# BUTSpeechFIT/DiariZen

Hardware: AMD Instinct MI355X
Metric: audio-seconds/s (RTF) for wavlm-large-s80 pipeline, 16 kHz mono (higher is better)
Workload: dtype f32 (operands split into 2 fp16 terms with exact power-of-two scaling = 22 significant bits, 3 fp16 MFMA products, fp32 accumulate: the error-corrected '3xFP16/3xTF32' scheme; kernels without an fp16 variant use the 3-term bf16 split)

## Files before the change

### diarizen_amd/_lib.py

```python
from __future__ import annotations

import ctypes as C
import os
from pathlib import Path

DZN_MAX_CONV = 8
DZN_MAX_LAYERS = 32
DZN_MAX_HEADS = 16

DZN_PREC_F32 = 0
DZN_PREC_BF16 = 1
DZN_PREC_F32_SPLIT = 2
DZN_PREC_F32_H2 = 3
DZN_PREC_F16 = 4

DZN_ACT_NONE, DZN_ACT_GELU, DZN_ACT_SWISH, DZN_ACT_RELU = 0, 1, 2, 3

DZN_F32, DZN_F64, DZN_I64 = 0, 1, 2

ERRORS = {0: "ok", -1: "invalid argument", -2: "out of memory", -3: "HIP runtime error",
          -4: "bad call order", -5: "missing state_dict key"}


class DznError(RuntimeError):
# ... 174 lines not shown
    sig("dzn_op_amax", i32, [vp, i64, vp, vp])
    sig("dzn_op_split_rows", i32, [vp, vp, i64, i64, i32, vp])
    sig("dzn_op_conv3x3_c32", i32, [vp, vp, vp, vp, vp, i32, i32, i32, i32, i32, vp])
    sig("dzn_op_resblock_ws", i32, [vp, vp, vp, vp, vp, vp, vp, vp, vp, f32, f32, i32, i32, i32, i32, vp])
    sig("dzn_op_resblock32_fused", i32, [vp, vp, vp, vp, vp, vp, vp, vp, vp, f32, f32, i32, i32, i32, vp])
    sig("dzn_op_set_resblock_np", i32, [i32])
    sig("dzn_op_set_attention_noskip", i32, [i32])
    sig("dzn_op_conv3x3_c32_h2", i32, [vp, vp, vp, vp, vp, vp, vp, vp, i32, i32, i32, i32, i32, vp])
    sig("dzn_op_conv3x3_c32_ex", i32, [vp, vp, vp, vp, vp, vp, vp, vp, i32, i32, i32, i32, i32, vp, vp, vp, vp])
    sig("dzn_op_resblock32_fused_ex", i32, [vp, vp, vp, vp, vp, vp, vp, vp, vp, vp, f32, f32, i32, i32, i32, i32, vp, vp, vp])
    sig("dzn_op_resblock_ws_ex", i32, [vp, vp, vp, vp, vp, vp, vp, vp, vp, vp, f32, f32, i32, i32, i32, i32, i32, vp, vp, vp])
    sig("dzn_op_layernorm", i32, [vp, i64, vp, i64, vp, vp, i64, i32, i32, f32, i32, vp])
    sig("dzn_op_gate", i32, [vp, i64, vp, vp, vp, vp, i64, i32, vp])
    sig("dzn_op_row_stats", i32, [vp, i64, i64, i32, f32, vp, vp])
    sig("dzn_op_gate_stats", i32, [vp, i64, vp, vp, vp, vp, vp, vp, vp, i64, i32, f32, vp])
    sig("dzn_op_attention_h2", i32, [vp, vp, vp, vp, vp, i32, i32, i32, i32, i32, i32, f32, vp, vp])
    sig("dzn_op_set_attention_qb", i32, [i32])
    sig("dzn_op_set_attention_prefetch", i32, [i32])
    sig("dzn_op_attention_planes", i32, [vp, vp, vp, vp, vp, i32, i32, i32, i32, i32, i32, f32, vp, vp, vp, vp])
    sig("dzn_op_attention", i32, [vp, vp, vp, vp, vp, i32, i32, i32, i32, i32, i32, f32, i32, vp])
    sig("dzn_op_glu_dwconv", i32, [vp, i64, vp, vp, vp, i64, i32, i32, i32, i32, vp])
    sig("dzn_op_classify", i32, [vp, i64, vp, vp, vp, i64, i32, i32, i32, vp, vp, vp, vp])
    sig("dzn_op_groupnorm_gelu", i32, [vp, vp, i32, i32, i32, i32, i64, vp, vp, f32, vp, vp, vp])
    sig("dzn_op_gn_stats_floats", i64, [i32, i32, i32, i32])
    sig("dzn_op_pad_rows", i32, [vp, vp, i32, i32, i32, i32, i32, vp])
    sig("dzn_op_ws_accum", i32, [vp, vp, f32, i32, i64, vp])
    sig("dzn_op_ws_sum", i32, [C.POINTER(vp), C.POINTER(f32), i32, vp, i64, vp])
    sig("dzn_op_col_scale", i32, [vp, i64, i32, i64, vp, vp])
    sig("dzn_op_layernorm_t", i32, [vp, i64, vp, i64, vp, vp, vp, i64, i32, i32, f32, i32, vp, i64, vp])
    sig("dzn_op_wave_stats", i32, [vp, i32, i32, f32, vp, vp])
# ... 3 lines not shown
    sig("dzn_op_log_cmn_gather", i32, [vp, i32, vp, i32, i32, i32, f32, vp])
    sig("dzn_op_stem_conv", i32, [vp, i32, i32, i32, i32, vp, vp, vp, vp, vp, vp, vp])
    sig("dzn_op_stats_pool", i32, [vp, i32, i32, i32, i32, vp, i32, i32, vp, vp, vp])
    sig("dzn_op_window_active", i32, [vp, i32, i32, vp, vp])
    sig("dzn_op_compact_active", i32, [vp, i32, vp, vp, vp, vp])
    _LIB = lib
    return lib


EXPORTED = [
    "dzn_create", "dzn_load_tensor", "dzn_finalize_weights", "dzn_num_frames",
    "dzn_segment_forward", "dzn_segment_forward_soft", "dzn_embed_forward", "dzn_embed_forward_strided", "dzn_prepare_masks", "dzn_speaker_count", "dzn_cluster_activations", "dzn_detect", "dzn_detect_range", "dzn_diarize_range", "dzn_speaker_scores", "dzn_debug_fetch", "dzn_embed_skip_stats", "dzn_num_ignored",
    "dzn_workspace_bytes", "dzn_last_error", "dzn_destroy", "dzn_version", "dzn_linkage_centroid", "dzn_cdist_cosine", "dzn_host_workspace_release",
    "dzn_host_workspace_bytes",
    "dzn_flac_info", "dzn_flac_decode", "dzn_resample", "dzn_resample_tile", "dzn_decode", "dzn_ingest_many", "dzn_gather_windows", "dzn_vbx_create", "dzn_vbx_stats", "dzn_vbx_estep", "dzn_vbx_gamma", "dzn_vbx_destroy",
    "dzn_op_gemm", "dzn_op_split_weights", "dzn_op_split_weights_h2", "dzn_op_split_weights_mx", "dzn_op_set_gemm_mx_cfg", "dzn_checked_status", "dzn_op_set_gemm_cfg", "dzn_op_amax", "dzn_op_conv3x3_c32", "dzn_op_conv3x3_c32_h2", "dzn_op_resblock32_fused", "dzn_op_resblock_ws", "dzn_op_set_resblock_np", "dzn_op_conv3x3_c32_ex", "dzn_op_resblock32_fused_ex", "dzn_op_resblock_ws_ex", "dzn_op_set_attention_noskip", "dzn_op_split_rows", "dzn_op_layernorm", "dzn_op_row_stats", "dzn_op_gate", "dzn_op_gate_stats", "dzn_op_attention", "dzn_op_attention_h2", "dzn_op_attention_planes", "dzn_op_set_attention_qb", "dzn_op_set_attention_prefetch",
    "dzn_profile_enable", "dzn_profile_collect", "dzn_profile_reserve", "dzn_op_relpos_bucket",
    "dzn_op_glu_dwconv", "dzn_op_classify", "dzn_op_groupnorm_gelu", "dzn_op_gn_stats_floats", "dzn_op_pad_rows", "dzn_op_ws_accum",
    "dzn_op_ws_sum", "dzn_op_col_scale", "dzn_op_layernorm_t", "dzn_op_wave_stats", "dzn_op_frame_prep", "dzn_op_power",
    "dzn_op_log_cmn", "dzn_op_log_cmn_gather", "dzn_op_stem_conv", "dzn_op_stats_pool", "dzn_op_window_active",
    "dzn_op_compact_active",
]


def profile_enable(on: bool) -> None:
    check(load().dzn_profile_enable(int(on)), None, "dzn_profile_enable")


def profile_reserve(n_events: int) -> None:
    check(load().dzn_profile_reserve(int(n_events)), None, "dzn_profile_reserve")

# ... 24 lines not shown
```

### diarizen_amd/csrc/attention.hip

```cpp
#include "common.h"

namespace {

template <bool BIAS>
__global__ __launch_bounds__(256) void attn_kernel(const float* __restrict__ qkv,
                                                   float* __restrict__ out,
                                                   const float* __restrict__ gate,
                                                   const float* __restrict__ table,
                                                   const int32_t* __restrict__ head_idx, int B,
                                                   int L, int h, int Htot, int ldqkv, int ldo,
                                                   float scale) {
  extern __shared__ __attribute__((aligned(16))) float smem_f[];
  float* sK = smem_f;
  float* sV = smem_f + 64 * 64;
  float* sT = smem_f + 2 * 64 * 64;

  const int tid = threadIdx.x, lane = tid & 63, wave = tid >> 6;
  const int lr = lane & 15, lq = lane >> 4;
  const int qt = blockIdx.x, j = blockIdx.y, b = blockIdx.z;
  const int64_t rowbase = (int64_t)b * L;
  const float* Qp = qkv + j * 64;
  const float* Kp = qkv + (h + j) * 64;
  const float* Vp = qkv + (2 * h + j) * 64;

// ... 256 lines not shown
        }
      }
      ta = dpp_add<0xB1, 0xF>(ta);
      ta = dpp_add<0x4E, 0xF>(ta);
      tb = dpp_add<0xB1, 0xF>(tb);
      tb = dpp_add<0x4E, 0xF>(tb);
      if (H < Htot && sub == 0) {
        const float ga = 1.0f / (1.0f + expf(-(ta + ba)));
        const float gb = 1.0f / (1.0f + expf(-(tb + bb)));
        gate[row * Htot + H] = ga * (gb * cst[H] - 1.0f) + 2.0f;
      }
    }
  }
}

}

int launch_gate_stats(const float* x, int64_t ldx, const float* gamma, const float* beta, const float* Wg,
                      const float* bg, const float* cst, float* gate, float* stats, int64_t rows, int Htot, float eps,
                      hipStream_t s) {
  if (rows <= 0) return DZN_OK;
  if (Htot < 1 || Htot > 16) return DZN_E_INVALID;
  int pid = prof_enabled() ? prof_begin(s, "gate_ln_stats", 0.0, (double)rows * Htot * 64 * 4.0) : -1;
  int64_t grid = cdiv64(rows, 4);
  grid = grid > 256 * 8 ? 256 * 8 : grid;
  hipLaunchKernelGGL(gate_stats_kernel<16>, dim3((unsigned)grid), dim3(256), 0, s, x, ldx, gamma, beta, Wg,
                     bg, cst, gate, stats, rows, Htot, eps);
  prof_end(pid, s);
  return hipGetLastError() == hipSuccess ? DZN_OK : DZN_E_HIP;
}
// ... 61 lines not shown
```

### diarizen_amd/csrc/common.h

```cpp
#pragma once
#include <hip/hip_runtime.h>
#include <stdint.h>
#include <math.h>
#include <string.h>
#include "../../include/dzn.h"
#include "../../include/dzn_ops.h"

typedef float f32x4 __attribute__((ext_vector_type(4)));
typedef __bf16 bf16x8 __attribute__((ext_vector_type(8)));
typedef __bf16 bf16x4 __attribute__((ext_vector_type(4)));
typedef unsigned short u16;

#define DZN_WAVE 64

template <int CTRL, int ROW_MASK>
__device__ __forceinline__ float dpp_add(float v) {
  const int t = __builtin_amdgcn_update_dpp(ROW_MASK == 0xF ? __float_as_int(v) : 0, __float_as_int(v), CTRL,
                                            ROW_MASK, 0xF, false);
  return v + __int_as_float(t);
}
__device__ __forceinline__ float wave_sum(float v) {
  v = dpp_add<0xB1, 0xF>(v);
  v = dpp_add<0x4E, 0xF>(v);
  v = dpp_add<0x124, 0xF>(v);
  v = dpp_add<0x128, 0xF>(v);
  v = dpp_add<0x142, 0xA>(v);
  v = dpp_add<0x143, 0xC>(v);
  return __int_as_float(__builtin_amdgcn_readlane(__float_as_int(v), 63));
}
__device__ __forceinline__ float wave_max(float v) {
#pragma unroll
  for (int o = 32; o > 0; o >>= 1) v = fmaxf(v, __shfl_xor(v, o, 64));
  return v;
}

__device__ __forceinline__ void track_amax_lane(float* tracker, float m) {
  if (m > 0.f) {
    const unsigned cur = __hip_atomic_load(reinterpret_cast<unsigned int*>(tracker), __ATOMIC_RELAXED, __HIP_MEMORY_SCOPE_AGENT);
    if (__float_as_uint(m) > cur) atomicMax(reinterpret_cast<unsigned int*>(tracker), __float_as_uint(m));
  }
}
__device__ __forceinline__ void track_amax(float* tracker, float wave_partial) {
  const float m = wave_max(wave_partial);
  if ((threadIdx.x & 63) == 0) track_amax_lane(tracker, m);
}

__device__ __forceinline__ float erf_as(float x) {
  const float ax = fabsf(x);
// ... 13 lines not shown
__device__ __forceinline__ float swishf_(float x) { return x * sigmoidf_(x); }

__device__ __forceinline__ float apply_act(float v, int act) {
  switch (act) {
    case DZN_ACT_GELU: return gelu_erf(v);
    case DZN_ACT_SWISH: return swishf_(v);
    case DZN_ACT_RELU: return fmaxf(v, 0.0f);
    default: return v;
  }
}

static inline bool prec_is_h2(int p) { return p == DZN_PREC_F32_H2 || p == DZN_PREC_F16; }
static inline bool prec_is_split(int p) { return p == DZN_PREC_F32_SPLIT || prec_is_h2(p); }

int launch_gemm(const dzn_gemm_desc& d, hipStream_t s);
int launch_gemm_split(const dzn_gemm_desc& d, hipStream_t s);
int launch_gemm_split_pre(const dzn_gemm_desc& d, hipStream_t s);
int launch_pad_rows_split3(const float* x, void* planes, int64_t plane_stride, int B, int L, int Lp, int pad, int D,
                           hipStream_t st, int cg = 0, int cgp = 0);
int launch_pad_rows_split2(const float* x, void* planes, int64_t plane_stride, int B, int L, int Lp, int pad, int D,
                           const float* amax, float* snapshot, hipStream_t st, int cg = 0, int cgp = 0);
int launch_split_weights(const float* W, int64_t rows, int K, int64_t ldw, void* W3, hipStream_t s);
int launch_split_weights_h2(const float* W, int64_t rows, int K, int64_t ldw, void* W2, float* col_scale, hipStream_t s);
int host_stage_stream(int device, hipStream_t* stream);
int host_state_lease(int device, size_t bytes, hipStream_t* stream, char** base);
void host_state_release(int device);
int launch_gemm_mx(const dzn_gemm_desc& d, hipStream_t s);
int launch_split_weights_mx(const float* W, int64_t rows, int K, int64_t ldw, void* Wmx, float* col_scale, hipStream_t s);
int launch_amax(const float* x, int64_t n, float* amax, hipStream_t s);
int launch_fill_u32(void* p, unsigned value, int64_t n, hipStream_t st);
int launch_stats_finalize(const float* partial, int64_t rows, int P, int C, float eps, float* stats, hipStream_t s);
int launch_layernorm(const float* x, int64_t ldx, float* y, int64_t ldy, const float* g,
                     const float* b, int64_t rows, int C, int Cpad, float eps, int gelu,
                     hipStream_t s);
int launch_layernorm_t(const float* x, int64_t ldx, float* y, int64_t ldy, const float* g, const float* b,
                       const float* post, int64_t rows, int C, int Cpad, float eps, int gelu, hipStream_t s,
                       float* amax = nullptr, int64_t amax_unit = 0);
int launch_row_stats(const float* x, int64_t ldx, int64_t rows, int C, float eps, float* stats, hipStream_t s);
int launch_gate_stats(const float* x, int64_t ldx, const float* gamma, const float* beta, const float* Wg,
                      const float* bg, const float* cst, float* gate, float* stats, int64_t rows, int Htot, float eps,
                      hipStream_t s);
int launch_wave_stats(const float* w, int B, int N, float eps, float* stats, hipStream_t s);
int launch_gate(const float* y, int64_t ldy, const float* Wg, const float* bg, const float* cst,
                float* gate, int64_t rows, int Htot, hipStream_t s);
int launch_attention_t(const float* qkv, float* out, const float* gate, const float* table,
                       const int32_t* head_idx, int B, int L, int h, int Htot, int ldqkv, int ldo,
                       float scale, hipStream_t s);
int launch_attention_split(const float* qkv, float* out, const float* gate, const float* table,
                           const int32_t* head_idx, int B, int L, int h, int Htot, int ldqkv, int ldo,
                           float scale, hipStream_t s, const float* amax = nullptr);
int launch_attention(const float* qkv, float* out, const float* gate, const float* table,
                     const int32_t* head_idx, int B, int L, int h, int Htot, int ldqkv, int ldo,
                     float scale, int precision, hipStream_t s);
int launch_attention_planes(const float* qkv, const void* planes, int64_t plane_stride, const float* kvs, int kv_ld, float* out,
                            const float* gate, const float* table, const int32_t* head_idx, int B, int L, int h, int Htot,
                            int ldqkv, int ldo, float scale, hipStream_t s, const float* amax);
// ... 122 lines not shown
```

### diarizen_amd/csrc/engine.cpp

```cpp
#include <algorithm>
#include <cmath>
#include <cstdio>
#include <cstdlib>
#include <map>
#include <set>
#include <stdexcept>
#include <string>
#include <vector>

#include "common.h"

#define HIPCHK(x)                                                                        \
  do {                                                                                   \
    hipError_t e_ = (x);                                                                 \
    if (e_ != hipSuccess) {                                                              \
      throw EngineError(e_ == hipErrorOutOfMemory ? DZN_E_NOMEM : DZN_E_HIP,             \
                        std::string(#x) + ": " + hipGetErrorString(e_));                 \
    }                                                                                    \
  } while (0)

namespace {

struct EngineError : std::runtime_error {
  int code;
// ... 27 lines not shown
struct NormLin {
  LNp ln;
  Lin lin;
  bool folded = false;
};

struct EncLayer {
  bool attn = false, ffn = false;
  bool pre_norm = false;
  int h = 0, F = 0, Fp = 0;
  LNp ln1, ln2;
  NormLin qkv, f1;
  Lin out, f2;
  float *Wg = nullptr, *bg = nullptr, *cst = nullptr;
  int32_t* head_idx = nullptr;
};

struct ConfLayer {
  NormLin ffn1_w1, ffn2_w1, qkv, pw1;
  Lin ffn1_w2, ffn2_w2, o, pw2;
  LNp out_ln;
  float *dw = nullptr, *dwb = nullptr;
};

struct ResConv {
  Lin l;
  int cin = 0, cout = 0, ksz = 3, stride = 1;
  int k2 = 0;
  float l1max = 0.f, bmax = 0.f;
};
// ... 483 lines not shown
        h->rel_embed = e.v;
      }
    }
    if (L.ffn) {
      L.F = c.ffn_dim[i];
      L.Fp = pad32(L.F);
      maxF = std::max(maxF, L.Fp);
      L.f1 = norm_lin_from_sd(h, lp + ".feed_forward.intermediate_dense", L.pre_norm ? lp + ".final_layer_norm" : "", fold, L.F, D,
                              L.Fp, D, &L.ln2);
      L.f2 = linear_from_sd(h, lp + ".feed_forward.output_dense", D, L.F, D, L.Fp);
    }
  }
  if (h->rel_embed.empty())
    throw EngineError(DZN_E_INVALID, "layer 0 must carry attention (rel_attn_embed lives there)");
  {
    const HostT& w = need(h, "weight_sum.weight");
    expect_numel(w, c.n_layers + 1, "weight_sum.weight");
    h->wsum_w = w.v;
  }
  const int A = h->A, Fh = h->Fh;
  h->proj = linear_from_sd(h, "proj", A, D, A, D);
  h->lnorm = ln_from_sd(h, "lnorm", A);
  h->conf.resize(c.conf_layers);
  for (int i = 0; i < c.conf_layers; ++i) {
    ConfLayer& L = h->conf[i];
    const std::string cp = "conformer.conformer_layer." + std::to_string(i);
    L.ffn1_w1 = norm_lin_from_sd(h, cp + ".ffn1.w_1", cp + ".ffn1.ln_norm", fold, Fh, A, Fh, A);
    L.ffn1_w2 = linear_from_sd(h, cp + ".ffn1.w_2", A, Fh, A, Fh);
    L.ffn2_w1 = norm_lin_from_sd(h, cp + ".ffn2.w_1", cp + ".ffn2.ln_norm", fold, Fh, A, Fh, A);
    L.ffn2_w2 = linear_from_sd(h, cp + ".ffn2.w_2", A, Fh, A, Fh);
// ... 399 lines not shown
  std::vector<float> t((size_t)Hn * W);
  for (int r = -(L - 1); r <= L - 1; ++r) {
    const int bk = relpos_bucket(r, h->cfg.num_buckets, h->cfg.max_distance);
    for (int hh = 0; hh < Hn; ++hh) t[(size_t)hh * W + (r + L - 1)] = h->rel_embed[(size_t)bk * Hn + hh];
  }
  if (!h->table) h->table = dalloc<float>(h, (int64_t)Hn * (2 * h->maxL - 1), false);
  HIPCHK(hipMemcpy(h->table, t.data(), t.size() * 4, hipMemcpyHostToDevice));
  h->table_L = L;
}

struct SegCall {
  H* h;
  hipStream_t st;
  int B, L;
  int64_t ML;
  float* am(int slot) const {
    return slot >= 0 && prec_is_h2(h->cfg.precision) ? h->amax + slot * (int64_t)h->cfg.max_batch : nullptr;
  }
  int conv_slot(const float* buf) const { return buf == h->bufA ? dzn_handle::AM_CONVA : dzn_handle::AM_CONVB; }
  void gemm(dzn_gemm_desc& d, F16Class cls) const {
    if (h->cfg.precision == DZN_PREC_F16) {
      if (!((h->sw.f16_mx >> cls) & 1)) d.Wmx = nullptr;
      if ((h->sw.f16_keep2 >> cls) & 1) d.precision = DZN_PREC_F32_H2;
    }
    if ((d.nz == 1 && d.M == (int)ML) || (d.a_rowoff && d.a_rowoff == h->pos_rowoff)) d.amax_unit = L;
    chk(launch_gemm(d, st), F16_CLASSES[cls]);
  }
};

dzn_gemm_desc norm_lin_desc(const SegCall& s, const NormLin& nl, const float* in, int in_slot, float* scratch, int scratch_slot,
// ... 143 lines not shown
    d.a_z0 = (int64_t)Lp * Da;
    d.c_z0 = (int64_t)L * D;
    d.alg_flops = 2.0 * (double)L * cg * h->posconv.Kt;
  }
  if (pre3) {
    d.A = reinterpret_cast<const float*>(h->xpad3);
    d.a_split3 = pre2 ? 2 : 1;
    d.a_plane = h->xpad3_plane;
    if (pre2) d.a_amax = s.am(dzn_handle::AM_XPAD);
  }
  d.c_amax = s.am(dzn_handle::AM_X);
  s.gemm(d, CLS_POSCONV);
  if (!c.layer_norm_first) ln_t(h->x, D, h->x, D, h->enc_ln, ML, D, 0, st, nullptr, s.am(dzn_handle::AM_X), L);
}

float* seg_encoder_layer(const SegCall& s, int i, float* xr, WsSumArgs& wsum) {
  H* h = s.h;
  hipStream_t st = s.st;
  const int L = s.L, D = h->D;
  const int64_t ML = s.ML;
  const EncLayer& Ly = h->layers[i];
  const bool defer = h->xl != nullptr;
  const float wl = h->wsum_w[i + 1];
  float* const own = defer ? h->xl + (int64_t)i * ML * D : xr;
  bool have_stats = false;
  if (Ly.attn) {
    const int hd = Ly.h * 64;
    const bool gs = Ly.qkv.folded;
    if (gs)
      chk(launch_gate_stats(xr, D, Ly.ln1.g, Ly.ln1.b, Ly.Wg, Ly.bg, Ly.cst, h->gate, h->rstat, ML, h->H, 1e-5f, st),
          "gate_stats");
    dzn_gemm_desc d = norm_lin_desc(s, Ly.qkv, xr, dzn_handle::AM_X, h->y, dzn_handle::AM_Y, h->qkv, 3 * hd, gs);
    if (!gs) chk(launch_gate(d.A, D, Ly.Wg, Ly.bg, Ly.cst, h->gate, ML, h->H, st), "gate");
    d.c_amax = s.am(dzn_handle::AM_QKV);
    const bool planes = h->kvp != nullptr && d.W2h && d.col_scale && d.a_amax;
    if (planes) {
      d.kv_planes = h->kvp;
      d.kv_plane_stride = (ML + 64) * (int64_t)(2 * hd);
      d.kv_scale = h->kvs;
      d.kv_ld = 2 * hd;
      d.kv_col0 = hd;
    }
    s.gemm(d, CLS_QKV);
    attention(s, &Ly, h->qkv, dzn_handle::AM_QKV, planes, h->ao);
// ... 14 lines not shown
  if (!Ly.pre_norm) ln_t(xr, D, xr, D, Ly.ln1, ML, D, 0, st, nullptr, s.am(dzn_handle::AM_X), L);
  if (Ly.ffn) {
    dzn_gemm_desc f1 = norm_lin_desc(s, Ly.f1, xr, dzn_handle::AM_X, h->y, dzn_handle::AM_Y, h->mid, Ly.Fp, have_stats);
    f1.act = DZN_ACT_GELU;
    f1.c_amax = s.am(dzn_handle::AM_MID);
    s.gemm(f1, CLS_FFN1);
    dzn_gemm_desc f2 = gd(h, h->mid, Ly.f2, own, ML, Ly.Fp, D);
    f2.R = xr;
    if (Ly.pre_norm && !defer) {
      f2.WS = h->ws;
      f2.ldws = D;
      f2.ws_w = wl;
    }
    f2.a_amax = s.am(dzn_handle::AM_MID);
    f2.c_amax = s.am(dzn_handle::AM_X);
    s.gemm(f2, CLS_FFN2);
    xr = own;
  } else if (Ly.pre_norm && !defer) {
    chk(launch_ws_accum(xr, h->ws, wl, 0, ML * D, st), "ws_accum");
  }
  if (!Ly.pre_norm) {
    ln_t(xr, D, xr, D, Ly.ln2, ML, D, 0, st, nullptr, s.am(dzn_handle::AM_X), L);
    chk(launch_ws_accum(xr, h->ws, wl, 0, ML * D, st), "ws_accum");
  } else if (defer) {
    wsum.x[wsum.n] = xr;
    wsum.w[wsum.n++] = wl;
  }
  if (h->sw.debug_taps) {
    const std::string nm = "layer" + std::to_string(i);
    tap(h, nm.c_str(), xr, ML, D, D, st);
  }
// ... 61 lines not shown

void seg_forward(H* h, const float* wave, int B, int N, float* d_logp, uint8_t* d_ml, float* d_soft, hipStream_t st) {
  const dzn_config& c = h->cfg;
  int T[DZN_MAX_CONV];
  {
    int n = N;
    for (int i = 0; i < c.n_conv; ++i) {
      n = conv_out(n, c.conv_k[i], c.conv_s[i]);
      T[i] = n;
    }
  }
  const int L = T[c.n_conv - 1];
  if (L < 1) throw EngineError(DZN_E_INVALID, "window too short");
  const int D = h->D, A = h->A;
  const int64_t ML = (int64_t)B * L, MB = c.max_batch;
  const SegCall s{h, st, B, L, ML};
  if (prec_is_h2(c.precision)) {
    chk(launch_fill_u32(h->amax, 0u, dzn_handle::AM_IMG0 * MB, st), "tracker reset");
    if (c.extractor_layer_norm && h->conv0_bound > 0.f) {
      uint32_t bits;
      memcpy(&bits, &h->conv0_bound, 4);
      chk(launch_fill_u32(h->amax + dzn_handle::AM_CONVA * MB, bits, B, st), "conv0 bound");
    }
  }
  seg_project(s, seg_conv_stack(s, wave, N, T));
  const bool defer = h->xl != nullptr;
  float* xr = h->x;
  WsSumArgs wsum{};
  if (defer) {
    wsum.x[wsum.n] = xr;
    wsum.w[wsum.n++] = h->wsum_w[0];
// ... 628 lines not shown
```

### diarizen_amd/csrc/gemm.hip

```cpp
#include "common.h"
#include "gemm_epilogue.h"
#include "gemm_launch.h"

namespace {

template <int BM, int BN, int WGM, int WGN>
__global__ __launch_bounds__(256) void gemm_kernel(const dzn_gemm_desc d) {
  static_assert(WGM * WGN == 4, "4 wavefronts per workgroup");
  constexpr int BK = 32;
  constexpr int KV = 4;
  constexpr int TM = BM / WGM, TN = BN / WGN;
  constexpr int MI = TM / 16, NI = TN / 16;
  constexpr int ACH = BM / 32;
  constexpr int WCH = BN / 32;
  constexpr int BUF = (BM + BN) * 128;

  extern __shared__ __attribute__((aligned(16))) unsigned char smem[];

  const int tid = threadIdx.x;
  const int lane = tid & 63;
  const int wave = tid >> 6;
  const int wm = wave / WGN, wn = wave % WGN;

  int tm, tn, z0, z1;
// ... 288 lines not shown
                    d.kv_col0 < d.N && !(d.kv_col0 & 63) && !(d.N & 63) && d.kv_ld == d.N - d.kv_col0 &&
                    !(d.kv_plane_stride & 3) && d.N > 32 && !g_gemm_cfg.get() && !gemm_no_h2();
    if (!ok) return DZN_E_INVALID;
  }
  if (d.A2) {
    const bool ok = d.a2_rowoff && d.k1 >= 128 && !(d.k1 & 63) && d.k2 > 0 && !(d.k2 & 31) && d.k1 + d.k2 <= d.K &&
                    d.K - (d.k1 + d.k2) < 64 && !(d.K & 31) && !(d.kc & 31) && !d.a_split3 && !d.kv_planes && !(d.a2_z0 & 3);
    if (!ok) return DZN_E_INVALID;
  }
  if (d.a_split3) return prec_is_split(d.precision) ? launch_gemm_split_pre(d, s) : DZN_E_INVALID;
  if (prec_is_split(d.precision) && d.W3 && !(d.K & 31) && !(d.kc & 31) && d.ldw == d.K)
    return launch_gemm_split(d, s);
  return launch_f32(d, s);
}

extern "C" int dzn_op_set_gemm_cfg(const char* cfg) {
  g_gemm_cfg.set(cfg);
  return DZN_OK;
}

extern "C" int dzn_op_gemm(const dzn_gemm_desc* d, void* stream) {
  if (!d || !d->A || !d->C) return DZN_E_INVALID;
  return launch_gemm(*d, reinterpret_cast<hipStream_t>(stream));
}
```

### diarizen_amd/csrc/gemm_launch.h

```cpp
#pragma once
#include <cstdio>
#include <cstdlib>

#include "common.h"

class TileOverride {
 public:
  explicit TileOverride(const char* env) : env_(env) {}
  const char* get() {
    if (!init_) set(getenv(env_));
    return buf_[0] ? buf_ : nullptr;
  }
  void set(const char* cfg) {
    init_ = true;
    snprintf(buf_, sizeof(buf_), "%s", cfg && strcmp(cfg, "auto") ? cfg : "");
  }

 private:
  const char* env_;
  char buf_[32] = {0};
  bool init_ = false;
};
inline TileOverride g_gemm_cfg{"DZN_GEMM_CFG"};
inline TileOverride g_gemm_mx_cfg{"DZN_GEMM_MX_CFG"};

inline bool gemm_no_h2() {
  static const bool v = getenv("DZN_NO_H2") != nullptr;
  return v;
}

inline int gemm_prof_begin(const dzn_gemm_desc& d, hipStream_t s, const char* tag, int BM, int BN, int w_bytes_per_elem) {
  if (!prof_enabled()) return -1;
  static const bool by_shape = getenv("DZN_PROFILE_SHAPES") != nullptr;
  char cls[64];
  if (by_shape) snprintf(cls, sizeof(cls), "gemm_%s_%dx%d M%d N%d K%d z%d", tag, BM, BN, d.M, d.N, d.K, d.nz);
  else snprintf(cls, sizeof(cls), "gemm_%s_%dx%d", tag, BM, BN);
  const double fl = d.alg_flops > 0 ? d.alg_flops * d.nz : 2.0 * d.M * d.N * d.K * d.nz;
  return prof_begin(s, cls, fl, gemm_alg_bytes(d, w_bytes_per_elem));
}

template <auto KERN, typename... Extra>
int launch_contraction(const dzn_gemm_desc& d, hipStream_t s, int threads, size_t lds, int BM, int BN, int WGN, const char* tag,
                       int w_bytes_per_elem, Extra... extra) {
  const int tilesM = (d.M + BM - 1) / BM, tilesN = (d.N + BN - 1) / BN;
  static unsigned long long attr_mask = 0;
  if (first_use_on_device(attr_mask))
    (void)hipFuncSetAttribute(reinterpret_cast<const void*>(KERN), hipFuncAttributeMaxDynamicSharedMemorySize, 160 * 1024);
  const int pid = gemm_prof_begin(d, s, tag, BM, BN, w_bytes_per_elem);
  hipLaunchKernelGGL(KERN, dim3(tilesM * tilesN, d.nz > 0 ? d.nz : 1, 1), dim3(threads), lds, s, d, extra...);
  prof_end(pid, s);
  if (hipGetLastError() != hipSuccess) return DZN_E_HIP;
  if (d.stat_partial && d.stat_final)
    return launch_stats_finalize(d.stat_partial, d.M, tilesN * WGN, d.stat_C, d.stat_eps, d.stat_final, s);
  return DZN_OK;
}

__device__ __forceinline__ bool gemm_tile(const dzn_gemm_desc& d, const int tilesN, int& tm, int& tn, int& z0, int& z1) {
  int t;
  {
    const int nwg = gridDim.x, bid = blockIdx.x;
    const int q = nwg >> 3, r = nwg & 7, xcd = bid & 7, idx = bid >> 3;
    t = (xcd < r ? xcd * (q + 1) : r * (q + 1) + (xcd - r) * q) + idx;
  }
  tm = t / tilesN;
  tn = t % tilesN;
  const int z = blockIdx.y;
// ... 9 lines not shown
```

### diarizen_amd/csrc/norm.hip

```cpp
#include <cstdint>
#include <initializer_list>

#include "common.h"

namespace {

template <int MAXI>
__global__ __launch_bounds__(256) void layernorm_kernel(const float* __restrict__ x, int64_t ldx,
                                                        float* __restrict__ y, int64_t ldy,
                                                        const float* __restrict__ gamma,
                                                        const float* __restrict__ beta,
                                                        const float* __restrict__ post, int64_t rows,
                                                        int C, int Cpad, float eps, int gelu,
                                                        float* __restrict__ amax_out, int64_t amax_unit, int rows_per_wave) {
  const int lane = threadIdx.x & 63, wave = threadIdx.x >> 6;
  const int64_t r0 = ((int64_t)blockIdx.x * 4 + wave) * rows_per_wave;
  float amax = 0.f;
  int64_t unit = amax_out && amax_unit > 0 && r0 < rows ? r0 / amax_unit : 0;
  for (int64_t row = r0; row < r0 + rows_per_wave && row < rows; ++row) {
    const float* xp = x + row * ldx;
    float v[MAXI];
    float sum = 0.f;
#pragma unroll
    for (int i = 0; i < MAXI; ++i) {
// ... 65 lines not shown
  }
  const float var = wave_sum(sq) / (float)C;
  if (lane == 0) *reinterpret_cast<float2*>(stats + 2 * row) = make_float2(mean, 1.0f / sqrtf(var + eps));
}

__global__ __launch_bounds__(256) void stats_finalize_kernel(const float2* __restrict__ part, int64_t rows, int P, int C,
                                                             float eps, float2* __restrict__ stats) {
  const int64_t r = (int64_t)blockIdx.x * 256 + threadIdx.x;
  if (r >= rows) return;
  double s = 0.0, q = 0.0;
  for (int p = 0; p < P; ++p) {
    const float2 v = part[r * P + p];
    s += (double)v.x;
    q += (double)v.y;
  }
  const double mean = s / C;
  double var = q / C - mean * mean;
  var = var > 0.0 ? var : 0.0;
  stats[r] = make_float2((float)mean, (float)(1.0 / sqrt(var + (double)eps)));
}

__global__ __launch_bounds__(1024) void wave_stats_kernel(const float* __restrict__ w, int N,
                                                          float eps, float* __restrict__ stats) {
  __shared__ float red[32];
  const int b = blockIdx.x;
  const float* p = w + (int64_t)b * N;
  const int tid = threadIdx.x, lane = tid & 63, wave = tid >> 6;
  float s = 0.f;
  for (int i = tid; i < N; i += 1024) s += p[i];
  s = wave_sum(s);
  if (lane == 0) red[wave] = s;
  __syncthreads();
  float tot = 0.f;
  for (int i = 0; i < 16; ++i) tot += red[i];
// ... 201 lines not shown
int launch_row_stats(const float* x, int64_t ldx, int64_t rows, int C, float eps, float* stats, hipStream_t s) {
  if (rows <= 0) return DZN_OK;
  if (C <= 0 || C > 2048) return DZN_E_INVALID;
  const unsigned grid = (unsigned)cdiv64(rows, 4);
  int pid = prof_enabled() ? prof_begin(s, "row_stats", 0.0, (double)rows * C * 4.0) : -1;
#define DZN_RS(MAXI) hipLaunchKernelGGL((row_stats_kernel<MAXI>), dim3(grid), dim3(256), 0, s, x, ldx, rows, C, eps, stats)
  if (C <= 256) DZN_RS(4);
  else if (C <= 512) DZN_RS(8);
  else if (C <= 1024) DZN_RS(16);
  else DZN_RS(32);
#undef DZN_RS
  prof_end(pid, s);
  return hipGetLastError() == hipSuccess ? DZN_OK : DZN_E_HIP;
}

extern "C" int dzn_op_row_stats(const float* x, int64_t ldx, int64_t rows, int32_t C, float eps, float* stats,
                                void* stream) {
  if (!x || !stats) return DZN_E_INVALID;
  return launch_row_stats(x, ldx, rows, C, eps, stats, reinterpret_cast<hipStream_t>(stream));
}

int launch_wave_stats(const float* w, int B, int N, float eps, float* stats, hipStream_t s) {
  ProfScope prof_scope_(s, "wave_stats", 0.0, (double)B * N * 4.0);
  if (B <= 0) return DZN_OK;
  hipLaunchKernelGGL(wave_stats_kernel, dim3(B), dim3(1024), 0, s, w, N, eps, stats);
  return hipGetLastError() == hipSuccess ? DZN_OK : DZN_E_HIP;
}

extern "C" int dzn_op_layernorm(const float* x, int64_t ldx, float* y, int64_t ldy,
                                const float* gamma, const float* beta, int64_t rows, int32_t C,
// ... 34 lines not shown
```

### diarizen_amd/engine.py

```python
from __future__ import annotations

import ctypes as C
from typing import Dict, Mapping, Optional

import numpy as np
import torch

from . import _lib
from ._lib import (DZN_F32, DZN_F64, DZN_I64, DZN_PREC_F32, DZN_PREC_F32_SPLIT, DznConfig,
                   check)
from .configs import EmbConfig, SegConfig

PRECISIONS = {"f32": DZN_PREC_F32, "fp32": DZN_PREC_F32,
              "f32s": DZN_PREC_F32_SPLIT, "f32_split": DZN_PREC_F32_SPLIT, "f32h": _lib.DZN_PREC_F32_H2,
              "f16": _lib.DZN_PREC_F16, "fp16": _lib.DZN_PREC_F16}


def make_dzn_config(seg: SegConfig, emb: Optional[EmbConfig], max_batch: int, max_samples: int,
                    precision: str = "f32h") -> DznConfig:
    c = DznConfig()
    c.struct_size = C.sizeof(DznConfig)
    c.precision = PRECISIONS[precision]
    c.max_batch = int(max_batch)
    c.max_samples = int(max_samples)
# ... 4 lines not shown
        c.conv_ch[i], c.conv_k[i], c.conv_s[i] = ch, k, s
    c.embed_dim = seg.embed_dim
    c.total_heads = seg.total_heads
    c.n_layers = seg.n_layers
    c.layer_norm_first = int(seg.layer_norm_first)
    c.pos_conv_kernel = seg.pos_conv_kernel
    c.pos_conv_groups = seg.pos_conv_groups
    c.num_buckets = seg.num_buckets
    c.max_distance = seg.max_distance
    for i in range(seg.n_layers):
        heads = seg.remaining_heads[i]
        c.use_attention[i] = int(len(heads) > 0)
        c.n_heads[i] = len(heads)
        for j, hd in enumerate(heads):
            c.head_idx[i][j] = hd
        c.use_ffn[i] = 1
        c.ffn_dim[i] = seg.ffn_dims[i]
    c.attention_in = seg.attention_in
    c.ffn_hidden = seg.ffn_hidden
    c.conf_heads = seg.conf_heads
    c.conf_layers = seg.conf_layers
    c.conf_kernel = seg.conf_kernel
    c.n_classes = seg.n_classes
    c.max_speakers_per_chunk = seg.max_speakers_per_chunk
    c.max_speakers_per_frame = seg.max_speakers_per_frame
    c.has_embedding = int(emb is not None)
    if emb is not None:
        c.embed_out_dim = emb.embed_dim
        c.num_mel_bins = emb.num_mel_bins
    return c

# ... 148 lines not shown
```

### diarizen_amd/ops.py

```python
from __future__ import annotations

import ctypes as C

import torch

from . import _lib
from ._lib import DznGemmDesc, check


def _stream() -> C.c_void_p:
    return C.c_void_p(torch.cuda.current_stream().cuda_stream)


def _p(t):
    return None if t is None else C.c_void_p(t.data_ptr())


def gemm(A, W, *, M=None, N=None, K=None, bias=None, R=None, C_out=None, WS=None, ws_w=0.0,
         ws_init=False, a_rowoff=None, c_rowoff=None, lda=None, kc=0, ldk=0, ldw=None, ldc=None,
         ldws=0, act=0, alpha=1.0, post_relu=False, nz=1, zdiv=1, zs=None, precision=0,
         W3=None, a_planes=None, ln_stats=None, ln_colsum=None, W2h=None, col_scale=None,
         a_amax=None, c_amax=None, amax_unit=None, want_row_stats=False, stat_eps=1e-5, mx=False, Wmx=None,
         col_scale_mx=None, kv_col0=None, A2=None, a2_rowoff=None, a2_z0=0, k1=0, k2=0, a2_amax=None,
         stat_bufs=None, kv_bufs=None, amax_guard=0):
# ... 342 lines not shown
    return out


def gate_stats(x, gamma, beta, Wg, bg, cst, eps=1e-5, out=None):
    lib = _lib.load()
    rows, Htot = x.shape[0], cst.numel()
    if out is None:
        out = (torch.empty((rows, Htot), device=x.device, dtype=torch.float32),
               torch.empty((rows, 2), device=x.device, dtype=torch.float32))
    gate_, stats = out
    check(lib.dzn_op_gate_stats(_p(x), x.stride(0), _p(gamma), _p(beta), _p(Wg), _p(bg), _p(cst), _p(gate_), _p(stats),
                                rows, Htot, eps, _stream()), what="dzn_op_gate_stats")
    return gate_, stats


def gate(y, Wg, bg, cst, out=None):
    lib = _lib.load()
    rows = y.shape[0]
    Htot = cst.numel()
    if out is None:
        out = torch.empty((rows, Htot), device=y.device, dtype=torch.float32)
    check(lib.dzn_op_gate(_p(y), y.stride(0), _p(Wg), _p(bg), _p(cst), _p(out), rows, Htot,
                          _stream()), what="dzn_op_gate")
    return out


def attention(qkv, B, L, h, *, gate=None, table=None, head_idx=None, Htot=0, scale=0.125,
              precision=0, out=None, ldqkv=None, ldo=None, amax=None):
    lib = _lib.load()
    ldqkv = qkv.stride(0) if ldqkv is None else int(ldqkv)
# ... 161 lines not shown
```

### include/dzn_ops.h

```cpp
#ifndef DZN_OPS_H_
#define DZN_OPS_H_

#include <stdint.h>

#ifdef __cplusplus
extern "C" {
#endif

#define DZN_ACT_NONE 0
#define DZN_ACT_GELU 1
#define DZN_ACT_SWISH 2
#define DZN_ACT_RELU 3

typedef struct dzn_gemm_desc {
  const float* A;
  const float* W;
  float* C;
  const float* bias;
  const float* R;
  float* WS;
  const int32_t* a_rowoff;
  const int32_t* c_rowoff;
  int32_t M, N, K;
  int64_t lda;
// ... 91 lines not shown
                          int32_t B, int32_t Hs, int32_t Ws, int32_t C, int32_t np, const int32_t* z_count,
                          const int32_t* z_list, void* stream);

int dzn_op_layernorm(const float* x, int64_t ldx, float* y, int64_t ldy, const float* gamma,
                     const float* beta, int64_t rows, int32_t C, int32_t Cpad, float eps,
                     int32_t gelu, void* stream);

int dzn_op_row_stats(const float* x, int64_t ldx, int64_t rows, int32_t C, float eps, float* stats, void* stream);

int dzn_op_gate(const float* y, int64_t ldy, const float* Wg, const float* bg, const float* cst,
                float* gate, int64_t rows, int32_t Htot, void* stream);

int dzn_op_gate_stats(const float* x, int64_t ldx, const float* gamma, const float* beta, const float* Wg,
                      const float* bg, const float* cst, float* gate, float* stats, int64_t rows, int32_t Htot,
                      float eps, void* stream);

int dzn_op_attention_h2(const float* qkv, float* out, const float* gate, const float* table, const int32_t* head_idx,
                        int32_t B, int32_t L, int32_t h, int32_t Htot, int32_t ldqkv, int32_t ldo, float scale,
                        const float* amax, void* stream);

int dzn_op_attention_planes(const float* qkv, float* out, const float* gate, const float* table, const int32_t* head_idx,
                            int32_t B, int32_t L, int32_t h, int32_t Htot, int32_t ldqkv, int32_t ldo, float scale,
                            const float* amax, void* planes, float* kvs, void* stream);

int dzn_op_set_attention_qb(int32_t query_blocks_per_wavefront);
int dzn_op_set_attention_prefetch(int32_t on);

int dzn_op_attention(const float* qkv, float* out, const float* gate, const float* table,
                     const int32_t* head_idx, int32_t B, int32_t L, int32_t h,
                     int32_t Htot, int32_t ldqkv, int32_t ldo, float scale,
// ... 47 lines not shown
```

Measured before the change: 1791.

## Feed FFN2 epilogue row-stat partials into next layer's gate/stats kernel

```diff
diff --git a/diarizen_amd/_lib.py b/diarizen_amd/_lib.py
--- a/diarizen_amd/_lib.py
+++ b/diarizen_amd/_lib.py
@@ -212,6 +212,8 @@
     sig("dzn_op_gate", i32, [vp, i64, vp, vp, vp, vp, i64, i32, vp])
     sig("dzn_op_row_stats", i32, [vp, i64, i64, i32, f32, vp, vp])
     sig("dzn_op_gate_stats", i32, [vp, i64, vp, vp, vp, vp, vp, vp, vp, i64, i32, f32, vp])
+    sig("dzn_op_gate_heads", i32, [vp, i64, vp, vp, vp, vp, vp, vp, i32, vp, i32, i32, f32, vp, vp, i64, i32, vp])
+    sig("dzn_op_stats_finalize", i32, [vp, i64, i32, i32, f32, vp, vp])
     sig("dzn_op_attention_h2", i32, [vp, vp, vp, vp, vp, i32, i32, i32, i32, i32, i32, f32, vp, vp])
     sig("dzn_op_set_attention_qb", i32, [i32])
     sig("dzn_op_set_attention_prefetch", i32, [i32])
@@ -245,7 +247,7 @@
     "dzn_workspace_bytes", "dzn_last_error", "dzn_destroy", "dzn_version", "dzn_linkage_centroid", "dzn_cdist_cosine", "dzn_host_workspace_release",
     "dzn_host_workspace_bytes",
     "dzn_flac_info", "dzn_flac_decode", "dzn_resample", "dzn_resample_tile", "dzn_decode", "dzn_ingest_many", "dzn_gather_windows", "dzn_vbx_create", "dzn_vbx_stats", "dzn_vbx_estep", "dzn_vbx_gamma", "dzn_vbx_destroy",
-    "dzn_op_gemm", "dzn_op_split_weights", "dzn_op_split_weights_h2", "dzn_op_split_weights_mx", "dzn_op_set_gemm_mx_cfg", "dzn_checked_status", "dzn_op_set_gemm_cfg", "dzn_op_amax", "dzn_op_conv3x3_c32", "dzn_op_conv3x3_c32_h2", "dzn_op_resblock32_fused", "dzn_op_resblock_ws", "dzn_op_set_resblock_np", "dzn_op_conv3x3_c32_ex", "dzn_op_resblock32_fused_ex", "dzn_op_resblock_ws_ex", "dzn_op_set_attention_noskip", "dzn_op_split_rows", "dzn_op_layernorm", "dzn_op_row_stats", "dzn_op_gate", "dzn_op_gate_stats", "dzn_op_attention", "dzn_op_attention_h2", "dzn_op_attention_planes", "dzn_op_set_attention_qb", "dzn_op_set_attention_prefetch",
+    "dzn_op_gemm", "dzn_op_split_weights", "dzn_op_split_weights_h2", "dzn_op_split_weights_mx", "dzn_op_set_gemm_mx_cfg", "dzn_checked_status", "dzn_op_set_gemm_cfg", "dzn_op_amax", "dzn_op_conv3x3_c32", "dzn_op_conv3x3_c32_h2", "dzn_op_resblock32_fused", "dzn_op_resblock_ws", "dzn_op_set_resblock_np", "dzn_op_conv3x3_c32_ex", "dzn_op_resblock32_fused_ex", "dzn_op_resblock_ws_ex", "dzn_op_set_attention_noskip", "dzn_op_split_rows", "dzn_op_layernorm", "dzn_op_row_stats", "dzn_op_gate", "dzn_op_gate_stats", "dzn_op_gate_heads", "dzn_op_stats_finalize", "dzn_op_attention", "dzn_op_attention_h2", "dzn_op_attention_planes", "dzn_op_set_attention_qb", "dzn_op_set_attention_prefetch",
     "dzn_profile_enable", "dzn_profile_collect", "dzn_profile_reserve", "dzn_op_relpos_bucket",
     "dzn_op_glu_dwconv", "dzn_op_classify", "dzn_op_groupnorm_gelu", "dzn_op_gn_stats_floats", "dzn_op_pad_rows", "dzn_op_ws_accum",
     "dzn_op_ws_sum", "dzn_op_col_scale", "dzn_op_layernorm_t", "dzn_op_wave_stats", "dzn_op_frame_prep", "dzn_op_power",
diff --git a/diarizen_amd/csrc/attention.hip b/diarizen_amd/csrc/attention.hip
--- a/diarizen_amd/csrc/attention.hip
+++ b/diarizen_amd/csrc/attention.hip
@@ -294,6 +294,147 @@
   }
 }
 
+template <bool VEC, int PT>
+__global__ __launch_bounds__(256, 4) void gate_heads_kernel(const float* __restrict__ x, int64_t ldx,
+                                                         const float* __restrict__ gamma, const float* __restrict__ beta,
+                                                         const float* __restrict__ Wg, const float* __restrict__ bg,
+                                                         const float* __restrict__ cst, const int32_t* __restrict__ head_idx,
+                                                         int h, const float2* __restrict__ part, int Prt, int C, float eps,
+                                                         float* __restrict__ gate, float* __restrict__ stats, int64_t rows,
+                                                         int Htot) {
+  __shared__ float sw[2 * 64 + 2];
+  if (threadIdx.x < 128) {
+    const int o0 = threadIdx.x < 64 ? 0 : 4, dch = threadIdx.x & 63;
+    sw[threadIdx.x] = (Wg[(o0 + 0) * 64 + dch] + Wg[(o0 + 1) * 64 + dch]) + (Wg[(o0 + 2) * 64 + dch] + Wg[(o0 + 3) * 64 + dch]);
+  } else if (threadIdx.x < 130) {
+    const int o0 = threadIdx.x == 128 ? 0 : 4;
+    sw[threadIdx.x] = (bg[o0] + bg[o0 + 1]) + (bg[o0 + 2] + bg[o0 + 3]);
+  }
+  __syncthreads();
+  const int P = PT > 0 ? PT : Prt;
+  const int lane = threadIdx.x & 63, wave = threadIdx.x >> 6;
+  const int sub = lane & 3, quad = lane >> 2;
+  float wa[16], wb[16];
+#pragma unroll
+  for (int j = 0; j < 16; ++j) {
+    wa[j] = sw[sub * 16 + j];
+    wb[j] = sw[64 + sub * 16 + j];
+  }
+  const float ba = sw[128], bb = sw[129];
+  const int rpp = 16 / h;
+  const int rslot = quad / h, hslot = quad - rslot * h;
+  int H = rslot < rpp ? head_idx[hslot] : -1;
+  if (H >= Htot) H = -1;
+  const bool kept = H >= 0;
+  const int e0 = kept ? H * 64 + sub * 16 : 0;
+  float gm[16], bt[16];
+#pragma unroll
+  for (int j = 0; j < 16; ++j) {
+    gm[j] = kept ? gamma[e0 + j] : 0.f;
+    bt[j] = kept ? beta[e0 + j] : 0.f;
+  }
+  const float cH = kept ? cst[H] : 0.f;
+  const bool writes_stats = rslot < rpp && hslot == 0 && sub == 0;
+  for (int64_t row0 = ((int64_t)blockIdx.x * 4 + wave) * rpp; row0 < rows; row0 += (int64_t)gridDim.x * 4 * rpp) {
+    const int64_t row = row0 + rslot;
+    const bool live = rslot < rpp && row < rows;
+    const bool work = live && kept;
+    float v[16];
+    if (work) {
+      const float* xp = x + row * ldx + e0;
+      if constexpr (VEC) {
+#pragma unroll
+        for (int j = 0; j < 4; ++j) {
+          const float4 t = *reinterpret_cast<const float4*>(xp + 4 * j);
+          v[4 * j] = t.x; v[4 * j + 1] = t.y; v[4 * j + 2] = t.z; v[4 * j + 3] = t.w;
+        }
+      } else {
+#pragma unroll
+        for (int j = 0; j < 16; ++j) v[j] = xp[j];
+      }
+    } else {
+#pragma unroll
+      for (int j = 0; j < 16; ++j) v[j] = 0.f;
+    }
+    double s = 0.0, q = 0.0;
+    if (live) {
+      const float2* pp = part + row * P;
+      if constexpr (PT > 0) {
+        float2 t[PT];
+#pragma unroll
+        for (int p = 0; p < PT; ++p) t[p] = pp[p];
+#pragma unroll
+        for (int p = 0; p < PT; ++p) {
+          s += (double)t[p].x;
+          q += (double)t[p].y;
+        }
+      } else {
+        for (int p = 0; p < P; ++p) {
+          const float2 t = pp[p];
+          s += (double)t.x;
+          q += (double)t.y;
+        }
+      }
+    }
+    const float2 st = stats_from_sums(s, q, C, eps);
+    const float mean = st.x, rstd = st.y;
+    if (live && writes_stats) *reinterpret_cast<float2*>(stats + 2 * row) = st;
+    float ta = 0.f, tb = 0.f;
+    if (work) {
+#pragma unroll
+      for (int j = 0; j < 16; ++j) {
+        const float y = (v[j] - mean) * rstd * gm[j] + bt[j];
+        ta = fmaf(y, wa[j], ta);
+        tb = fmaf(y, wb[j], tb);
+      }
+    }
+    ta = dpp_add<0xB1, 0xF>(ta);
+    ta = dpp_add<0x4E, 0xF>(ta);
+    tb = dpp_add<0xB1, 0xF>(tb);
+    tb = dpp_add<0x4E, 0xF>(tb);
+    if (work && sub == 0) {
+      const float ga = 1.0f / (1.0f + expf(-(ta + ba)));
+      const float gb = 1.0f / (1.0f + expf(-(tb + bb)));
+      gate[row * Htot + H] = ga * (gb * cH - 1.0f) + 2.0f;
+    }
+  }
+}
+
+}
+
+int launch_gate_heads(const float* x, int64_t ldx, const float* gamma, const float* beta, const float* Wg, const float* bg,
+                      const float* cst, const int32_t* head_idx, int h, const float* stat_partial, int P, int C, float eps,
+                      float* gate, float* stats, int64_t rows, int Htot, hipStream_t s) {
+  if (Htot < 1 || Htot > 16 || h < 1 || h > Htot || P < 1 || P > 32 || C < Htot * 64) return DZN_E_INVALID;
+  if (rows <= 0) return DZN_OK;
+  int pid = prof_enabled() ? prof_begin(s, "gate_heads", 0.0, (double)rows * (h * 64 * 4.0 + P * 8.0 + 8.0 + h * 4.0)) : -1;
+  int64_t grid = cdiv64(cdiv64(rows, 16 / h), 4);
+  grid = grid > 256 * 4 ? 256 * 4 : grid;
+  const bool vec = ((reinterpret_cast<uintptr_t>(x) | (uintptr_t)(ldx * 4)) & 15) == 0;
+#define DZN_GH(VECV, PTV)                                                                                                   \
+  hipLaunchKernelGGL((gate_heads_kernel<VECV, PTV>), dim3((unsigned)grid), dim3(256), 0, s, x, ldx, gamma, beta, Wg, bg, cst, \
+                     head_idx, h, reinterpret_cast<const float2*>(stat_partial), P, C, eps, gate, stats, rows, Htot)
+#define DZN_GHP(PTV)   \
+  do {                 \
+    if (vec) DZN_GH(true, PTV); \
+    else DZN_GH(false, PTV);    \
+  } while (0)
+  if (P == 8) DZN_GHP(8);
+  else if (P == 16) DZN_GHP(16);
+  else DZN_GHP(0);
+#undef DZN_GHP
+#undef DZN_GH
+  prof_end(pid, s);
+  return hipGetLastError() == hipSuccess ? DZN_OK : DZN_E_HIP;
+}
+
+extern "C" int dzn_op_gate_heads(const float* x, int64_t ldx, const float* gamma, const float* beta, const float* Wg,
+                                 const float* bg, const float* cst, const int32_t* head_idx, int32_t h,
+                                 const float* stat_partial, int32_t P, int32_t C, float eps, float* gate, float* stats,
+                                 int64_t rows, int32_t Htot, void* stream) {
+  if (!x || !gamma || !beta || !Wg || !bg || !cst || !head_idx || !stat_partial || !gate || !stats) return DZN_E_INVALID;
+  return launch_gate_heads(x, ldx, gamma, beta, Wg, bg, cst, head_idx, h, stat_partial, P, C, eps, gate, stats, rows, Htot,
+                           reinterpret_cast<hipStream_t>(stream));
 }
 
 int launch_gate_stats(const float* x, int64_t ldx, const float* gamma, const float* beta, const float* Wg,
diff --git a/diarizen_amd/csrc/common.h b/diarizen_amd/csrc/common.h
--- a/diarizen_amd/csrc/common.h
+++ b/diarizen_amd/csrc/common.h
@@ -32,6 +32,13 @@
 #pragma unroll
   for (int o = 32; o > 0; o >>= 1) v = fmaxf(v, __shfl_xor(v, o, 64));
   return v;
+}
+
+__device__ __forceinline__ float2 stats_from_sums(double s, double q, int C, float eps) {
+  const double mean = s / C;
+  double var = q / C - mean * mean;
+  var = var > 0.0 ? var : 0.0;
+  return make_float2((float)mean, (float)(1.0 / sqrt(var + (double)eps)));
 }
 
 __device__ __forceinline__ void track_amax_lane(float* tracker, float m) {
@@ -75,6 +82,7 @@
 static inline bool prec_is_split(int p) { return p == DZN_PREC_F32_SPLIT || prec_is_h2(p); }
 
 int launch_gemm(const dzn_gemm_desc& d, hipStream_t s);
+int gemm_stat_partials_last();
 int launch_gemm_split(const dzn_gemm_desc& d, hipStream_t s);
 int launch_gemm_split_pre(const dzn_gemm_desc& d, hipStream_t s);
 int launch_pad_rows_split3(const float* x, void* planes, int64_t plane_stride, int B, int L, int Lp, int pad, int D,
@@ -101,6 +109,9 @@
 int launch_gate_stats(const float* x, int64_t ldx, const float* gamma, const float* beta, const float* Wg,
                       const float* bg, const float* cst, float* gate, float* stats, int64_t rows, int Htot, float eps,
                       hipStream_t s);
+int launch_gate_heads(const float* x, int64_t ldx, const float* gamma, const float* beta, const float* Wg, const float* bg,
+                      const float* cst, const int32_t* head_idx, int h, const float* stat_partial, int P, int C, float eps,
+                      float* gate, float* stats, int64_t rows, int Htot, hipStream_t s);
 int launch_wave_stats(const float* w, int B, int N, float eps, float* stats, hipStream_t s);
 int launch_gate(const float* y, int64_t ldy, const float* Wg, const float* bg, const float* cst,
                 float* gate, int64_t rows, int Htot, hipStream_t s);
diff --git a/diarizen_amd/csrc/engine.cpp b/diarizen_amd/csrc/engine.cpp
--- a/diarizen_amd/csrc/engine.cpp
+++ b/diarizen_amd/csrc/engine.cpp
@@ -65,6 +65,7 @@
   Lin out, f2;
   float *Wg = nullptr, *bg = nullptr, *cst = nullptr;
   int32_t* head_idx = nullptr;
+  bool stats_in = false;
 };
 
 struct ConfLayer {
@@ -578,6 +579,20 @@
   if (h->rel_embed.empty())
     throw EngineError(DZN_E_INVALID, "layer 0 must carry attention (rel_attn_embed lives there)");
   {
+    bool any = false;
+    for (int i = 0; i < c.n_layers; ++i) {
+      EncLayer& L = h->layers[i];
+      if (!h->sw.epilogue_stats) break;
+      any = any || (L.attn && L.ffn && L.f1.folded);
+      if (i == 0 || !L.pre_norm || !h->layers[i - 1].ffn) continue;
+      L.stats_in = L.attn ? (L.qkv.folded && D == h->H * 64 && h->H <= 16) : (L.ffn && L.f1.folded);
+      any = any || L.stats_in;
+    }
+    if (any && 2 * ((D + 63) / 64) > 32)
+      throw EngineError(DZN_E_INVALID, "encoder_embed_dim > 1024: the epilogue's row statistics need more than 32 partials per row "
+                                       "(DZN_NO_EPILOGUE_STATS=1 runs without them)");
+  }
+  {
     const HostT& w = need(h, "weight_sum.weight");
     expect_numel(w, c.n_layers + 1, "weight_sum.weight");
     h->wsum_w = w.v;
@@ -1007,6 +1022,7 @@
   hipStream_t st;
   int B, L;
   int64_t ML;
+  int stat_P = 0;
   float* am(int slot) const {
     return slot >= 0 && prec_is_h2(h->cfg.precision) ? h->amax + slot * (int64_t)h->cfg.max_batch : nullptr;
   }
@@ -1180,7 +1196,7 @@
   if (!c.layer_norm_first) ln_t(h->x, D, h->x, D, h->enc_ln, ML, D, 0, st, nullptr, s.am(dzn_handle::AM_X), L);
 }
 
-float* seg_encoder_layer(const SegCall& s, int i, float* xr, WsSumArgs& wsum) {
+float* seg_encoder_layer(SegCall& s, int i, float* xr, WsSumArgs& wsum) {
   H* h = s.h;
   hipStream_t st = s.st;
   const int L = s.L, D = h->D;
@@ -1189,11 +1205,15 @@
   const bool defer = h->xl != nullptr;
   const float wl = h->wsum_w[i + 1];
   float* const own = defer ? h->xl + (int64_t)i * ML * D : xr;
-  bool have_stats = false;
+  bool have_stats = Ly.stats_in && !Ly.attn;
   if (Ly.attn) {
     const int hd = Ly.h * 64;
     const bool gs = Ly.qkv.folded;
-    if (gs)
+    if (gs && Ly.stats_in)
+      chk(launch_gate_heads(xr, D, Ly.ln1.g, Ly.ln1.b, Ly.Wg, Ly.bg, Ly.cst, Ly.head_idx, Ly.h, h->spart, s.stat_P, D, 1e-5f,
+                            h->gate, h->rstat, ML, h->H, st),
+          "gate_heads");
+    else if (gs)
       chk(launch_gate_stats(xr, D, Ly.ln1.g, Ly.ln1.b, Ly.Wg, Ly.bg, Ly.cst, h->gate, h->rstat, ML, h->H, 1e-5f, st),
           "gate_stats");
     dzn_gemm_desc d = norm_lin_desc(s, Ly.qkv, xr, dzn_handle::AM_X, h->y, dzn_handle::AM_Y, h->qkv, 3 * hd, gs);
@@ -1238,7 +1258,15 @@
     }
     f2.a_amax = s.am(dzn_handle::AM_MID);
     f2.c_amax = s.am(dzn_handle::AM_X);
+    const EncLayer* next = i + 1 < h->cfg.n_layers ? &h->layers[i + 1] : nullptr;
+    if (next && next->stats_in) {
+      f2.stat_partial = h->spart;
+      f2.stat_final = next->attn ? nullptr : h->rstat;
+      f2.stat_C = D;
+      f2.stat_eps = 1e-5f;
+    }
     s.gemm(f2, CLS_FFN2);
+    if (f2.stat_partial) s.stat_P = gemm_stat_partials_last();
     xr = own;
   } else if (Ly.pre_norm && !defer) {
     chk(launch_ws_accum(xr, h->ws, wl, 0, ML * D, st), "ws_accum");
@@ -1330,7 +1358,7 @@
   if (L < 1) throw EngineError(DZN_E_INVALID, "window too short");
   const int D = h->D, A = h->A;
   const int64_t ML = (int64_t)B * L, MB = c.max_batch;
-  const SegCall s{h, st, B, L, ML};
+  SegCall s{h, st, B, L, ML};
   if (prec_is_h2(c.precision)) {
     chk(launch_fill_u32(h->amax, 0u, dzn_handle::AM_IMG0 * MB, st), "tracker reset");
     if (c.extractor_layer_norm && h->conv0_bound > 0.f) {
diff --git a/diarizen_amd/csrc/gemm.hip b/diarizen_amd/csrc/gemm.hip
--- a/diarizen_amd/csrc/gemm.hip
+++ b/diarizen_amd/csrc/gemm.hip
@@ -326,6 +326,8 @@
   return launch_f32(d, s);
 }
 
+int gemm_stat_partials_last() { return g_stat_partials_last; }
+
 extern "C" int dzn_op_set_gemm_cfg(const char* cfg) {
   g_gemm_cfg.set(cfg);
   return DZN_OK;
diff --git a/diarizen_amd/csrc/gemm_launch.h b/diarizen_amd/csrc/gemm_launch.h
--- a/diarizen_amd/csrc/gemm_launch.h
+++ b/diarizen_amd/csrc/gemm_launch.h
@@ -29,6 +29,8 @@
   return v;
 }
 
+inline thread_local int g_stat_partials_last = 0;
+
 inline int gemm_prof_begin(const dzn_gemm_desc& d, hipStream_t s, const char* tag, int BM, int BN, int w_bytes_per_elem) {
   if (!prof_enabled()) return -1;
   static const bool by_shape = getenv("DZN_PROFILE_SHAPES") != nullptr;
@@ -50,6 +52,7 @@
   hipLaunchKernelGGL(KERN, dim3(tilesM * tilesN, d.nz > 0 ? d.nz : 1, 1), dim3(threads), lds, s, d, extra...);
   prof_end(pid, s);
   if (hipGetLastError() != hipSuccess) return DZN_E_HIP;
+  if (d.stat_partial) g_stat_partials_last = tilesN * WGN;
   if (d.stat_partial && d.stat_final)
     return launch_stats_finalize(d.stat_partial, d.M, tilesN * WGN, d.stat_C, d.stat_eps, d.stat_final, s);
   return DZN_OK;
diff --git a/diarizen_amd/csrc/norm.hip b/diarizen_amd/csrc/norm.hip
--- a/diarizen_amd/csrc/norm.hip
+++ b/diarizen_amd/csrc/norm.hip
@@ -103,10 +103,7 @@
     s += (double)v.x;
     q += (double)v.y;
   }
-  const double mean = s / C;
-  double var = q / C - mean * mean;
-  var = var > 0.0 ? var : 0.0;
-  stats[r] = make_float2((float)mean, (float)(1.0 / sqrt(var + (double)eps)));
+  stats[r] = stats_from_sums(s, q, C, eps);
 }
 
 __global__ __launch_bounds__(1024) void wave_stats_kernel(const float* __restrict__ w, int N,
@@ -338,6 +335,12 @@
   return hipGetLastError() == hipSuccess ? DZN_OK : DZN_E_HIP;
 }
 
+extern "C" int dzn_op_stats_finalize(const float* partial, int64_t rows, int32_t P, int32_t C, float eps, float* stats,
+                                     void* stream) {
+  if (!partial || !stats) return DZN_E_INVALID;
+  return launch_stats_finalize(partial, rows, P, C, eps, stats, reinterpret_cast<hipStream_t>(stream));
+}
+
 extern "C" int dzn_op_row_stats(const float* x, int64_t ldx, int64_t rows, int32_t C, float eps, float* stats,
                                 void* stream) {
   if (!x || !stats) return DZN_E_INVALID;
diff --git a/diarizen_amd/engine.py b/diarizen_amd/engine.py
--- a/diarizen_amd/engine.py
+++ b/diarizen_amd/engine.py
@@ -42,7 +42,7 @@
         c.n_heads[i] = len(heads)
         for j, hd in enumerate(heads):
             c.head_idx[i][j] = hd
-        c.use_ffn[i] = 1
+        c.use_ffn[i] = int(seg.ffn_dims[i] > 0)
         c.ffn_dim[i] = seg.ffn_dims[i]
     c.attention_in = seg.attention_in
     c.ffn_hidden = seg.ffn_hidden
diff --git a/diarizen_amd/ops.py b/diarizen_amd/ops.py
--- a/diarizen_amd/ops.py
+++ b/diarizen_amd/ops.py
@@ -380,6 +380,30 @@
     return gate_, stats
 
 
+def stats_finalize(partial, C, eps=1e-5, out=None):
+    lib = _lib.load()
+    rows, P = partial.shape[0], partial.shape[1]
+    assert partial.is_contiguous() and partial.dtype == torch.float32 and partial.shape[2] == 2
+    if out is None:
+        out = torch.empty((rows, 2), device=partial.device, dtype=torch.float32)
+    check(lib.dzn_op_stats_finalize(_p(partial), rows, P, C, eps, _p(out), _stream()), what="dzn_op_stats_finalize")
+    return out
+
+
+def gate_heads(x, gamma, beta, Wg, bg, cst, head_idx, partial, eps=1e-5, out=None, h=None, P=None):
+    lib = _lib.load()
+    rows, Htot = x.shape[0], cst.numel()
+    assert head_idx.dtype == torch.int32 and partial.dtype == torch.float32 and partial.is_contiguous()
+    if out is None:
+        out = (torch.empty((rows, Htot), device=x.device, dtype=torch.float32),
+               torch.empty((rows, 2), device=x.device, dtype=torch.float32))
+    gate_, stats = out
+    check(lib.dzn_op_gate_heads(_p(x), x.stride(0), _p(gamma), _p(beta), _p(Wg), _p(bg), _p(cst), _p(head_idx),
+                                head_idx.numel() if h is None else h, _p(partial), partial.shape[1] if P is None else P,
+                                Htot * 64, eps, _p(gate_), _p(stats), rows, Htot, _stream()), what="dzn_op_gate_heads")
+    return gate_, stats
+
+
 def gate(y, Wg, bg, cst, out=None):
     lib = _lib.load()
     rows = y.shape[0]
diff --git a/include/dzn_ops.h b/include/dzn_ops.h
--- a/include/dzn_ops.h
+++ b/include/dzn_ops.h
@@ -129,6 +129,11 @@
 int dzn_op_gate_stats(const float* x, int64_t ldx, const float* gamma, const float* beta, const float* Wg,
                       const float* bg, const float* cst, float* gate, float* stats, int64_t rows, int32_t Htot,
                       float eps, void* stream);
+int dzn_op_stats_finalize(const float* partial, int64_t rows, int32_t P, int32_t C, float eps, float* stats, void* stream);
+int dzn_op_gate_heads(const float* x, int64_t ldx, const float* gamma, const float* beta, const float* Wg,
+                      const float* bg, const float* cst, const int32_t* head_idx, int32_t h, const float* stat_partial,
+                      int32_t P, int32_t C, float eps, float* gate, float* stats, int64_t rows, int32_t Htot,
+                      void* stream);
 
 int dzn_op_attention_h2(const float* qkv, float* out, const float* gate, const float* table, const int32_t* head_idx,
                         int32_t B, int32_t L, int32_t h, int32_t Htot, int32_t ldqkv, int32_t ldo, float scale,
```

New measurement: 1810 (median of 6 runs). +1.0%, better.
